# BAMresearch/McSAS

Hardware: AMD Instinct MI355X
Metric: MC accept/reject steps/sec (whole node) (higher is better)
Workload: dtype f64; 1 GPU; Sphere, synthetic 512 q-points x 400 contribs, 50 reps on this rank (50 in all), 20000 MC steps per chain per launch, convergenceCriterion=0, one analysis on the chip at a time; reps_total=50, reps_per_gpu=50, ranks_seen=1, streams=1, exec_mode=pipeline, waves_per_chain=1, q_per_lane=8, window=192, launches=108, cached_rows=True

## Files before the change

### mcsas_amd/csrc/pipe_gram.h

```cpp
#pragma once
#include "pipe_layout.h"

namespace mcsas {

#define PIPE_LDS_BARRIER() do { asm volatile("s_waitcnt lgkmcnt(0)" ::: "memory"); __builtin_amdgcn_s_barrier(); asm volatile("" ::: "memory"); } while (0)

typedef double v4f64 __attribute__((ext_vector_type(4)));
typedef double v2f64 __attribute__((ext_vector_type(2)));


template <int T>
__device__ __forceinline__ void pipe_gram_store(int tsel, int idx, double sum, int W, MCSAS_GLOBAL double *gout, MCSAS_GLOBAL double *scal_sub = nullptr) {
    int ti = 0, tgi = 0, tgj = 0;
#pragma unroll
    for (int gi = 0; gi < T; ++gi)
#pragma unroll
        for (int gj = gi; gj < T; ++gj) { if (ti == tsel) { tgi = gi; tgj = gj; } ++ti; }
    const int i = 4 * (idx >> 6) + ((idx & 63) >> 4), j = idx & 15;
    const int ar = 16 * tgi + i, kc = 16 * tgj + j;
    if (ar < W && kc < W) {
        gout[(size_t)ar * W + kc] = sum;
        if (scal_sub && ar == kc) scal_sub[ar * 4 + 2] = sum;
    }
}

template <int QPL, int T, bool PACK>
__device__ __forceinline__ void pipe_gram_mfma_lds(const double *drows, int dstr, int nvalid, const double *lw, int gw,
                                                   v4f64 (&acc)[PACK ? 2 : T * (T + 1) / 2]) {
    const int lane = threadIdx.x & 63;
    const int m = lane & 15, kk = lane >> 4;
    constexpr int NT = PACK ? 2 : T * (T + 1) / 2;
    constexpr int NL = PACK ? 3 : T;
    constexpr int SLICE = 64 * QPL / PIPE_WAVES;
    static_assert(SLICE >= 8, "too many waves for this q count");
    const int qs = gw * SLICE + kk * 2;
#pragma unroll
    for (int i = 0; i < NT; ++i) acc[i] = (v4f64){0., 0., 0., 0.};
    const double *rowp[NL];
    bool rowok[NL];
#pragma unroll
    for (int gi = 0; gi < NL; ++gi) {
        const int rr = PACK ? (gi == 0 ? m : gi == 1 ? 8 + m : (m < 8 ? m : m + 8)) : 16 * gi + m;
        rowok[gi] = rr < nvalid;
        rowp[gi] = drows + (size_t)(rowok[gi] ? rr : 0) * dstr + qs;
    }
#pragma unroll
    for (int sp = 0; sp < SLICE / 8; ++sp) {
        v2f64 av[NL], bv[NL];
        const v2f64 wv = *reinterpret_cast<const v2f64 *>(lw + qs + 8 * sp);
#pragma unroll
        for (int gi = 0; gi < NL; ++gi) {
            const v2f64 x = *reinterpret_cast<const v2f64 *>(rowp[gi] + 8 * sp);
            av[gi] = rowok[gi] ? x : (v2f64){0., 0.};
            bv[gi] = av[gi] * wv;
        }
        if constexpr (PACK) {
            acc[0] = __builtin_amdgcn_mfma_f64_16x16x4f64(av[0].x, bv[1].x, acc[0], 0, 0, 0);
            acc[1] = __builtin_amdgcn_mfma_f64_16x16x4f64(av[2].x, bv[2].x, acc[1], 0, 0, 0);
            acc[0] = __builtin_amdgcn_mfma_f64_16x16x4f64(av[0].y, bv[1].y, acc[0], 0, 0, 0);
            acc[1] = __builtin_amdgcn_mfma_f64_16x16x4f64(av[2].y, bv[2].y, acc[1], 0, 0, 0);
        } else {
            int ti = 0;
#pragma unroll
            for (int gi = 0; gi < T; ++gi)
#pragma unroll
                for (int gj = gi; gj < T; ++gj) {
                    acc[ti] = __builtin_amdgcn_mfma_f64_16x16x4f64(av[gi].x, bv[gj].x, acc[ti], 0, 0, 0);
                    acc[ti] = __builtin_amdgcn_mfma_f64_16x16x4f64(av[gi].y, bv[gj].y, acc[ti], 0, 0, 0);
                    ++ti;
                }
        }
    }
}

__device__ __forceinline__ void pipe_gram_store_pack(int tsel, int idx, double sum, MCSAS_GLOBAL double *gout, MCSAS_GLOBAL double *scal_sub) {
    const int i = 4 * (idx >> 6) + ((idx & 63) >> 4), j = idx & 15;
    if (tsel == 0) {
        gout[(size_t)i * 24 + 8 + j] = sum;
        if (i == 8 + j) scal_sub[i * 4 + 2] = sum;
    } else if ((i < 8) == (j < 8)) {
        const int ar = i < 8 ? i : i + 8, kc = j < 8 ? j : j + 8;
        gout[(size_t)ar * 24 + kc] = sum;
        if (ar == kc) scal_sub[ar * 4 + 2] = sum;
    }
}

template <int QPL, int T, bool PACK>
__device__ __forceinline__ void pipe_prod_gram_lds_t(const double *drows, int dstr, int W, int nvalid, const double *lw,
                                                     double *gred, MCSAS_GLOBAL double *gout, MCSAS_GLOBAL double *scal_sub) {
    const int tid = threadIdx.x, lane = tid & 63, wave = __builtin_amdgcn_readfirstlane(tid >> 6);
    constexpr int NT = PACK ? 2 : T * (T + 1) / 2;
    v4f64 acc[NT];
    pipe_gram_mfma_lds<QPL, T, PACK>(drows, dstr, nvalid, lw, wave, acc);
    constexpr int TPR = PIPE_GRAM_TILES_PER_ROUND;
#pragma unroll
    for (int r0 = 0; r0 < NT; r0 += TPR) {
#pragma unroll
        for (int u = 0; u < TPR; ++u)
            if (r0 + u < NT) {
#pragma unroll
                for (int r = 0; r < 4; ++r) gred[((size_t)(wave * TPR + u) * 4 + r) * 64 + lane] = acc[r0 + u < NT ? r0 + u : 0][r];
            }
        PIPE_LDS_BARRIER();
        {
            const int u = tid >> 8, idx = tid & 255;
            const int tsel = r0 + u;
            if (tsel < NT) {
                double sum = 0.;
#pragma unroll
                for (int v = 0; v < PIPE_WAVES; ++v) sum += gred[(size_t)(v * TPR + u) * 256 + idx];
                if constexpr (PACK) pipe_gram_store_pack(tsel, idx, sum, gout, scal_sub);
                else pipe_gram_store<T>(tsel, idx, sum, W, gout, scal_sub);
            }
        }
        if (r0 + TPR < NT) PIPE_LDS_BARRIER();
    }
}

template <int QPL>
__device__ __forceinline__ void pipe_prod_gram_lds(const double *drows, int dstr, int W, int nvalid, const double *lw,
                                                   double *gred, MCSAS_GLOBAL double *gout, MCSAS_GLOBAL double *scal_sub) {
    if (W == 24) { pipe_prod_gram_lds_t<QPL, 2, true>(drows, dstr, W, nvalid, lw, gred, gout, scal_sub); return; }
    switch ((W + 15) >> 4) {
        case 1: pipe_prod_gram_lds_t<QPL, 1, false>(drows, dstr, W, nvalid, lw, gred, gout, scal_sub); break;
        case 2: pipe_prod_gram_lds_t<QPL, 2, false>(drows, dstr, W, nvalid, lw, gred, gout, scal_sub); break;
        case 3: pipe_prod_gram_lds_t<QPL, 3, false>(drows, dstr, W, nvalid, lw, gred, gout, scal_sub); break;
        default: pipe_prod_gram_lds_t<QPL, 4, false>(drows, dstr, W, nvalid, lw, gred, gout, scal_sub); break;
    }
}

#ifdef MCSAS_TUNING

template <int QPL, int T, bool PACK>
__device__ __forceinline__ void pipe_gram_units(const MCSAS_GLOBAL double *drows, int qpad, int nvalid, const double *lw, int gw,
                                                int u0, int u1, v4f64 (&acc)[PIPE_GRAM_NT_MAX]) {
    static_assert(T <= 2, "at most two 16-row groups per sub-window");
    const int lane = threadIdx.x & 63;
    const int m = lane & 15, kk = lane >> 4;
    constexpr int NL = PACK ? 3 : T;
    constexpr int SLICE = 64 * QPL / PIPE_WAVES;
    static_assert(SLICE >= 8, "too many waves for this q count");
    const int qs = gw * SLICE + kk * 2;
    if (u0 == 0) {
#pragma unroll
        for (int i = 0; i < PIPE_GRAM_NT_MAX; ++i) acc[i] = (v4f64){0., 0., 0., 0.};
    }
    const MCSAS_GLOBAL double *rowp[NL];
    bool rowok[NL];
#pragma unroll
    for (int gi = 0; gi < NL; ++gi) {
        const int rr = PACK ? (gi == 0 ? m : gi == 1 ? 8 + m : (m < 8 ? m : m + 8)) : 16 * gi + m;
        rowok[gi] = rr < nvalid;
        rowp[gi] = drows + (size_t)(rowok[gi] ? rr : 0) * qpad + qs;
    }
    v2f64 cur[NL], nxt[NL];
#pragma unroll
    for (int gi = 0; gi < NL; ++gi) cur[gi] = *(const MCSAS_GLOBAL v2f64 *)(rowp[gi] + 8 * u0);
    for (int u = u0; u < u1; ++u) {
        const int un = u + 1 < u1 ? u + 1 : u;
#pragma unroll
        for (int gi = 0; gi < NL; ++gi) nxt[gi] = *(const MCSAS_GLOBAL v2f64 *)(rowp[gi] + 8 * un);
        const v2f64 wv = *reinterpret_cast<const v2f64 *>(lw + qs + 8 * u);
        v2f64 av[NL], bv[NL];
#pragma unroll
        for (int gi = 0; gi < NL; ++gi) {
            av[gi] = rowok[gi] ? cur[gi] : (v2f64){0., 0.};
            bv[gi] = av[gi] * wv;
        }
        if constexpr (PACK) {
            acc[0] = __builtin_amdgcn_mfma_f64_16x16x4f64(av[0].x, bv[1].x, acc[0], 0, 0, 0);
            acc[1] = __builtin_amdgcn_mfma_f64_16x16x4f64(av[2].x, bv[2].x, acc[1], 0, 0, 0);
            acc[0] = __builtin_amdgcn_mfma_f64_16x16x4f64(av[0].y, bv[1].y, acc[0], 0, 0, 0);
            acc[1] = __builtin_amdgcn_mfma_f64_16x16x4f64(av[2].y, bv[2].y, acc[1], 0, 0, 0);
        } else {
            int ti = 0;
#pragma unroll
            for (int gi = 0; gi < T; ++gi)
#pragma unroll
                for (int gj = gi; gj < T; ++gj) { acc[ti] = __builtin_amdgcn_mfma_f64_16x16x4f64(av[gi].x, bv[gj].x, acc[ti], 0, 0, 0); ++ti; }
            ti = 0;
#pragma unroll
            for (int gi = 0; gi < T; ++gi)
#pragma unroll
                for (int gj = gi; gj < T; ++gj) { acc[ti] = __builtin_amdgcn_mfma_f64_16x16x4f64(av[gi].y, bv[gj].y, acc[ti], 0, 0, 0); ++ti; }
        }
#pragma unroll
        for (int gi = 0; gi < NL; ++gi) cur[gi] = nxt[gi];
    }
}

constexpr int PIPE_GRAM_PREF = 12;
template <int T, bool PACK> struct PipeGramScheme {
    static constexpr int NL = PACK ? 3 : T;
    static constexpr int UCAP = PIPE_GRAM_PREF / NL;
};
template <int QPL, int T, bool PACK>
__device__ __forceinline__ void pipe_gram_fetch(const MCSAS_GLOBAL double *drows, int qpad, int nvalid, int gw, int u0, int n,
                                                v2f64 (&G)[PIPE_GRAM_PREF]) {
    const int lane = threadIdx.x & 63;
    const int m = lane & 15, kk = lane >> 4;
    constexpr int NL = PipeGramScheme<T, PACK>::NL, UCAP = PipeGramScheme<T, PACK>::UCAP;
    constexpr int SLICE = 64 * QPL / PIPE_WAVES;
    const int qs = gw * SLICE + kk * 2;
#pragma unroll
    for (int gi = 0; gi < NL; ++gi) {
        const int rr = PACK ? (gi == 0 ? m : gi == 1 ? 8 + m : (m < 8 ? m : m + 8)) : 16 * gi + m;
        const MCSAS_GLOBAL double *rowp = drows + (size_t)(rr < nvalid ? rr : 0) * qpad + qs;
#pragma unroll
        for (int i = 0; i < UCAP; ++i) {
            const int u = u0 + (i < n ? i : n - 1);
            G[i * NL + gi] = *(const MCSAS_GLOBAL v2f64 *)(rowp + 8 * u);
        }
    }
}
template <int QPL, int T, bool PACK>
__device__ __forceinline__ void pipe_gram_consume(const v2f64 (&G)[PIPE_GRAM_PREF], int nvalid, const double *lw, int gw, int u0, int n,
                                                  v4f64 (&acc)[PIPE_GRAM_NT_MAX]) {
    const int lane = threadIdx.x & 63;
    const int m = lane & 15, kk = lane >> 4;
    constexpr int NL = PipeGramScheme<T, PACK>::NL, UCAP = PipeGramScheme<T, PACK>::UCAP;
    constexpr int SLICE = 64 * QPL / PIPE_WAVES;
    const int qs = gw * SLICE + kk * 2;
    if (u0 == 0) {
#pragma unroll
        for (int i = 0; i < PIPE_GRAM_NT_MAX; ++i) acc[i] = (v4f64){0., 0., 0., 0.};
    }
    bool rowok[NL];
#pragma unroll
    for (int gi = 0; gi < NL; ++gi) {
        const int rr = PACK ? (gi == 0 ? m : gi == 1 ? 8 + m : (m < 8 ? m : m + 8)) : 16 * gi + m;
        rowok[gi] = rr < nvalid;
    }
#pragma unroll
    for (int i = 0; i < UCAP; ++i)
        if (i < n) {
            const v2f64 wv = *reinterpret_cast<const v2f64 *>(lw + qs + 8 * (u0 + i));
            v2f64 av[NL], bv[NL];
#pragma unroll
            for (int gi = 0; gi < NL; ++gi) {
                av[gi] = rowok[gi] ? G[i * NL + gi] : (v2f64){0., 0.};
                bv[gi] = av[gi] * wv;
            }
            if constexpr (PACK) {
                acc[0] = __builtin_amdgcn_mfma_f64_16x16x4f64(av[0].x, bv[1].x, acc[0], 0, 0, 0);
                acc[1] = __builtin_amdgcn_mfma_f64_16x16x4f64(av[2].x, bv[2].x, acc[1], 0, 0, 0);
                acc[0] = __builtin_amdgcn_mfma_f64_16x16x4f64(av[0].y, bv[1].y, acc[0], 0, 0, 0);
                acc[1] = __builtin_amdgcn_mfma_f64_16x16x4f64(av[2].y, bv[2].y, acc[1], 0, 0, 0);
            } else {
                int ti = 0;
#pragma unroll
                for (int gi = 0; gi < T; ++gi)
#pragma unroll
                    for (int gj = gi; gj < T; ++gj) { acc[ti] = __builtin_amdgcn_mfma_f64_16x16x4f64(av[gi].x, bv[gj].x, acc[ti], 0, 0, 0); ++ti; }
                ti = 0;
#pragma unroll
                for (int gi = 0; gi < T; ++gi)
#pragma unroll
                    for (int gj = gi; gj < T; ++gj) { acc[ti] = __builtin_amdgcn_mfma_f64_16x16x4f64(av[gi].y, bv[gj].y, acc[ti], 0, 0, 0); ++ti; }
            }
        }
}

__device__ __forceinline__ int pipe_gram_tiles(int W) { return W == 24 ? 2 : (W <= 16 ? 1 : 3); }

__device__ __forceinline__ void pipe_gram_park(const v4f64 (&acc)[PIPE_GRAM_NT_MAX], int nt, double *gred, int wave, int lane) {
#pragma unroll
    for (int ti = 0; ti < PIPE_GRAM_NT_MAX; ++ti)
        if (ti < nt) {
#pragma unroll
            for (int r = 0; r < 4; ++r) gred[((size_t)(wave * PIPE_GRAM_NT_MAX + ti) * 4 + r) * 64 + lane] = acc[ti][r];
        }
}

__device__ __forceinline__ void pipe_gram_sum_store(int W, const double *gred, MCSAS_GLOBAL double *gout, MCSAS_GLOBAL double *scal_sub) {
    const int tid = threadIdx.x;
    const int nt = pipe_gram_tiles(W);
    for (int e = tid; e < nt * 256; e += PIPE_BLOCK) {
        const int ti = e >> 8, idx = e & 255;
        double sum = 0.;
#pragma unroll
        for (int v = 0; v < PIPE_WAVES; ++v) sum += gred[(size_t)(v * PIPE_GRAM_NT_MAX + ti) * 256 + idx];
        const int i = 4 * (idx >> 6) + ((idx & 63) >> 4), j = idx & 15;
        int ar = -1, kc = -1;
        if (W == 24) {
            if (ti == 0) { ar = i; kc = 8 + j; }
            else if ((i < 8) == (j < 8)) { ar = i < 8 ? i : i + 8; kc = j < 8 ? j : j + 8; }
        } else {
            const int tgi = ti == 2 ? 1 : 0, tgj = ti == 0 ? 0 : 1;
            ar = 16 * tgi + i; kc = 16 * tgj + j;
        }
        if (ar >= 0 && ar < W && kc < W) {
            gout[(size_t)ar * W + kc] = sum;
            if (ar == kc) scal_sub[ar * 4 + 2] = sum;
        }
    }
}
#endif

}
```

### mcsas_amd/csrc/pipe_prod.h

```cpp
#pragma once
#include "pipe_rowq.h"
#include <type_traits>

namespace mcsas {

#define PIPE_PIN_ROW(arr) do { _Pragma("unroll") for (int j_ = 0; j_ < QPL; ++j_) asm volatile("" : "+v"(arr[j_])); } while (0)

#ifdef MCSAS_STAMPS
#define PIPE_TL_SLOT(pa, i) (pa).timeline[((size_t)blockIdx.x * 8 + (threadIdx.x >> 6)) * PIPE_TL_WORDS + 4 + (i)]
#define PIPE_TL_PUT(pa, t, i, val) do { if ((pa).timeline && (t) - 1 == (pa).timeline_tick && (threadIdx.x & 63) == 0) PIPE_TL_SLOT(pa, i) = (val); } while (0)
#define PIPE_TL_CLOCK(var) const uint64_t var = wall_clock64()
#else
#define PIPE_TL_PUT(pa, t, i, val) do {} while (0)
#define PIPE_TL_CLOCK(var) do {} while (0)
#endif
#define PIPE_TL_WRITE(pa, t, i) PIPE_TL_PUT(pa, t, i, wall_clock64())
#define PIPE_TLX_MARK(pa, t, i) PIPE_TL_WRITE(pa, t, 18 + (i))
#define PIPE_TL_MARK(pa, t, i) PIPE_TL_WRITE(pa, t, i)

template <int M> constexpr bool pipe_light_model_v = Contrib<M>::ROW_CLASS == 0;
template <int M>
__device__ __forceinline__ double pipe_point_intensity(const Contrib<M> &c, double q, double q3inv, const double *tab) {
    if constexpr (M == MCSAS_MODEL_SPHERE) return c.fast ? c.intensity_fast(q, q3inv) : c.intensity(q, tab);
    else return c.intensity(q, tab);
}

template <int QPL>
__device__ __forceinline__ void load_row_pairs(const MCSAS_GLOBAL double *row, int lane, double (&r)[QPL]) {
    if constexpr (QPL >= 2) {
#pragma unroll
        for (int c = 0; c < QPL / 2; ++c) {
            const v2f64 v = *(const MCSAS_GLOBAL v2f64 *)(row + 128 * c + 2 * lane);
            r[2 * c] = v.x; r[2 * c + 1] = v.y;
        }
    } else {
        r[0] = row[lane];
    }
}
template <int QPL>
__device__ __forceinline__ void load_row_pairs_lds(const double *row, int lane, double (&r)[QPL]) {
    if constexpr (QPL >= 2) {
#pragma unroll
        for (int c = 0; c < QPL / 2; ++c) {
            const v2f64 v = *reinterpret_cast<const v2f64 *>(row + 128 * c + 2 * lane);
            r[2 * c] = v.x; r[2 * c + 1] = v.y;
        }
    } else {
        r[0] = row[lane];
    }
}

template <int M, int QPL, bool RQ>
__device__ __forceinline__ void pipe_prod_block(const PipeArgs &pa, const PipeHot &hot, double *lds, int rep, int by, int gy, int t) {
    const ChainArgs &a = pa.c;
    const int tid = threadIdx.x, lane = tid & 63, wave = tid >> 6;
    constexpr int WPB = PIPE_BLOCK / 64;
    const int N = hot.n_contrib, P = hot.n_active, qpad = hot.qpad, Kb = hot.kb;
    const int64_t max_iter = hot.max_iter;
    constexpr int QTB = (QPL * 64 + PIPE_BLOCK - 1) / PIPE_BLOCK;
    double tq[QTB], tw[QTB], twI[QTB], tq3[QTB];
#pragma unroll
    for (int x = 0; x < QTB; ++x) {
        const int i = tid + PIPE_BLOCK * x < qpad ? tid + PIPE_BLOCK * x : 0;
        tq[x] = glb(hot.q)[i]; tw[x] = glb(hot.w)[i]; twI[x] = glb(hot.wI)[i]; tq3[x] = glb(hot.q3inv)[i];
    }
    PIPE_TL_CLOCK(c_entry);
    const PipeSnap sn = load_snap(&hot.chains[rep].snap[t & 1]);
    const bool own = sn.alive && t >= sn.t_init;
    if (!own && !(RQ && pa.g.help)) return;
    PIPE_TL_CLOCK(c_snap);

    double *lq = lds, *lw = lds + qpad, *lwI = lds + 2 * qpad, *lq3 = lds + 3 * qpad, *tab = lds + 4 * qpad;
#pragma unroll
    for (int x = 0; x < QTB; ++x) {
        const int i = tid + PIPE_BLOCK * x;
        if (i < qpad) { lq[i] = tq[x]; lw[i] = tw[x]; lwI[i] = twI[x]; lq3[i] = tq3[x]; }
    }
    PIPE_TL_CLOCK(c_tab);
    Contrib<M>::fill_table(a.model, tab, tid, PIPE_BLOCK);
    if (tid == 0) {
        *reinterpret_cast<int32_t *>(lds + pa.g.gram_off + 16) = 0;
        *reinterpret_cast<int32_t *>(lds + pa.g.gram_off) = 0;
    }
    __syncthreads();
    PIPE_TL_CLOCK(c_bar);
    PIPE_TL_PUT(pa, t, 22, c_entry); PIPE_TL_PUT(pa, t, 23, c_snap); PIPE_TL_PUT(pa, t, 24, c_tab); PIPE_TL_PUT(pa, t, 25, c_bar);
    const QTables qt = make_qtables<M>(a.model, lq, lq3, tab);
    if constexpr (RQ) { pipe_prod_rowq<M, QPL>(pa, hot, lds, qt, rep, by, gy, t, sn, own); return; }
    auto rset = glb(a.rset) + (size_t)rep * N * P;
    auto cache = glb(a.cache) + (size_t)rep * a.cache_rows * qpad;
    const DrawSource src{a.replay ? a.replay + (size_t)rep * a.replay_len : nullptr, a.replay_len, a.seed,
                         (uint32_t)(a.rep_offset + rep)};
    auto slot_of = glb(pa.slot_of) + (size_t)rep * N;
    auto stage = glb(pa.stage_slot) + (size_t)rep * 2 * Kb;
    auto row_valid = glb(pa.row_valid) + (size_t)rep * N;
    const int gw = by * WPB + wave, nw = gy * WPB;

    if (t == sn.t_init) {
        for (int i = tid + by * PIPE_BLOCK; i < N; i += PIPE_BLOCK * gy) { slot_of[i] = i; row_valid[i] = 1; }
        for (int i = tid + by * PIPE_BLOCK; i < 2 * Kb; i += PIPE_BLOCK * gy) stage[i] = N + i;
        int ovf = 0;
        for (int nb = 0; nb < N; nb += nw * WAVE) {
            const int n = nb + lane * nw + gw;
            double row[MCSAS_MAX_ACTIVE] = {0., 0., 0., 0.};
            if (n < N) {
#pragma unroll
                for (int p = 0; p < MCSAS_MAX_ACTIVE; ++p)
                    if (p < P) {
                        if (a.start_from_min) row[p] = a.start_value[p];
                        else {
                            double u = src.at(sn.init_base + (uint64_t)p * N + n, ovf);
                            row[p] = gen_transform(a.gen_kind[p], u) * (a.gen_hi[p] - a.gen_lo[p]) + a.gen_lo[p];
                        }
                        rset[(size_t)n * P + p] = row[p];
                    }
            } else {
#pragma unroll
                for (int p = 0; p < MCSAS_MAX_ACTIVE; ++p) row[p] = a.gen_lo[p] > 0. ? a.gen_lo[p] : 1e-9;
            }
            Contrib<M> mine;
            mine.prepare(a.model, row);
            for (int l = 0; l < WAVE; ++l) {
                const int nn = nb + l * nw + gw;
                if (nn >= N) break;
                const Contrib<M> c = mine.bcast(__builtin_amdgcn_readfirstlane(l));
                double it[QPL];
                RowEval<M, QPL>::run(c, qt, lane, it);
#pragma unroll
                for (int j = 0; j < QPL; ++j) cache[(size_t)nn * qpad + lane + WAVE * j] = it[j];
            }
        }
        if (__any(ovf) && lane == 0) atomicOr(&pa.chains[rep].overflow, 1);
        return;
    }

    if (MCSAS_TUNE_BITS(a) & 16) return;
    if constexpr (pipe_light_model_v<M>) if (pa.g.overlap || pa.g.gram_lds) {
        const int W = pa.g.w, nsb = pa.g.sub_per_block, BR = nsb * W;
        const int buf = t & 1;
        const int64_t w = (int64_t)t - sn.t_init - 1;
        const int64_t sb0 = w * Kb + (int64_t)by * BR;
        auto dwin = glb(pa.dwin) + ((size_t)rep * 2 + buf) * Kb * qpad;
        auto scal = glb(pa.scal) + ((size_t)rep * 2 + buf) * Kb * 4;
        auto pval = glb(pa.pval) + ((size_t)rep * 2 + buf) * Kb * MCSAS_MAX_ACTIVE;
        auto povf = glb(pa.povf) + ((size_t)rep * 2 + buf) * Kb;
        auto gwin = glb(pa.gwin) + ((size_t)rep * 2 + buf) * Kb * W;
        double *gred = lds + pa.g.gram_off + 16;
        const bool no_gram = MCSAS_TUNE_BITS(a) & 64;
        const bool lazy = pa.g.lazy_rows;
        PIPE_TLX_MARK(pa, t, 0);
        constexpr int CON = PIPE_PROP_DOUBLES;
        static_assert(sizeof(Contrib<M>) <= 8 * (CON - 1) && sizeof(Contrib<M>) % 8 == 0, "Contrib record");
        int32_t *stl = reinterpret_cast<int32_t *>(gred);
        double *scon = gred + 64;
        auto stale_push = [&](int r, const Contrib<M> &c) {
            const int e = atomicAdd(&stl[0], 1);
            stl[1 + e] = r;
            double tmp[CON] = {};
            __builtin_memcpy(tmp, &c, sizeof(Contrib<M>));
#pragma unroll
            for (int i = 0; i < (int)(sizeof(Contrib<M>) / 8); ++i) scon[e * CON + i] = tmp[i];
        };
        auto stale_refresh = [&]() {
            PIPE_LDS_BARRIER();
            const int nst = stl[0];
            for (int i = 0; i < nst; ++i) {
                const int r = stl[1 + i];
                Contrib<M> c;
                {
                    double tmp[CON];
#pragma unroll
                    for (int x = 0; x < (int)(sizeof(Contrib<M>) / 8); ++x) tmp[x] = scon[i * CON + x];
                    __builtin_memcpy(&c, tmp, sizeof(Contrib<M>));
                }
#pragma unroll
                for (int x = 0; x < QTB; ++x) {
                    const int iq = tid + PIPE_BLOCK * x;
                    if (iq < qpad) cache[(size_t)r * qpad + iq] = pipe_point_intensity<M>(c, lq[iq], lq3[iq], tab);
                }
                if (tid == 0) row_valid[r] = 1;
            }
            if (nst) __syncthreads();
            else PIPE_LDS_BARRIER();
        };
        auto nvalid_of = [&](int ss) {
            const int64_t left = max_iter - (w * Kb + (int64_t)(by * nsb + ss) * W);
            return left >= W ? W : (left > 0 ? (int)left : 0);
        };
        if (pa.g.gram_lds) {
            const int dstr = qpad + PIPE_DROW_PAD;
            double *dbuf = lds + pa.g.drow_off;
            double *prec = lds + pa.g.rec_off;
            int32_t *claim = reinterpret_cast<int32_t *>(lds + pa.g.gram_off);
            auto take = [&]() {
                int v = 0;
                if (lane == 0) v = __hip_atomic_fetch_add(claim, 1, __ATOMIC_RELAXED, __HIP_MEMORY_SCOPE_WORKGROUP);
                return __builtin_amdgcn_readfirstlane(v);
            };
            int kc = take();
            const int kk = tid & 63;
            const int64_t sl = sb0 + kk;
            const bool prop_thr = tid < BR, old_thr = lazy && tid >= 64 && tid - 64 < BR && sl < max_iter;
            const int rk = (int)(sl % N);
            double prow[MCSAS_MAX_ACTIVE] = {0., 0., 0., 0.};
            int stale_r = -1, pov = 0;
            if (old_thr) {
                const int v = row_valid[rk];
#pragma unroll
                for (int p = 0; p < MCSAS_MAX_ACTIVE; ++p) if (p < P) prow[p] = rset[(size_t)rk * P + p];
                if (!v) stale_r = rk;
            }
#pragma unroll
            for (int p = 0; p < MCSAS_MAX_ACTIVE; ++p)
                if (p < P) {
                    double u = 0.5;
                    if (prop_thr && sl < max_iter) u = src.at(sn.step_base + (uint64_t)sl * P + p, pov);
                    const double pv = gen_transform(a.gen_kind[p], u) * (a.gen_hi[p] - a.gen_lo[p]) + a.gen_lo[p];
                    if (!old_thr) prow[p] = pv;
                }
            Contrib<M> prop;
            prop.prepare(a.model, prow);
            PIPE_TLX_MARK(pa, t, 1);
            if (prop_thr) {
                double tmp[CON] = {};
                __builtin_memcpy(tmp, &prop, sizeof(Contrib<M>));
#pragma unroll
                for (int i = 0; i < (int)(sizeof(Contrib<M>) / 8); ++i) prec[kk * CON + i] = tmp[i];
                if (!lazy) {
                    int32_t *slots = reinterpret_cast<int32_t *>(prec + kk * CON + CON - 1);
                    slots[0] = slot_of[rk]; slots[1] = stage[buf * Kb + by * BR + kk];
                }
                const int k = by * BR + kk;
#pragma unroll
                for (int p = 0; p < MCSAS_MAX_ACTIVE; ++p) if (p < P) pval[k * MCSAS_MAX_ACTIVE + p] = prow[p];
                povf[k] = pov;
            }
            if (stale_r >= 0) stale_push(stale_r, prop);
            if (lazy) stale_refresh();
            else PIPE_LDS_BARRIER();
            PIPE_TLX_MARK(pa, t, 2);
            PIPE_TLX_MARK(pa, t, 3);
            const int r0 = (int)(sb0 % N);
            auto oslot_of = [&](int k) {
                if (lazy) return r0 + k < N ? r0 + k : r0 + k - N;
                return __builtin_amdgcn_readfirstlane(reinterpret_cast<const int32_t *>(prec + k * CON + CON - 1)[0]);
            };
            double ocur[QPL], onext[QPL];
            {
                const auto orow0 = cache + (size_t)oslot_of(kc < BR ? kc : BR - 1) * qpad + lane;
#pragma unroll
                for (int j = 0; j < QPL; ++j) ocur[j] = orow0[WAVE * j];
            }
            PIPE_PIN_ROW(ocur);
#ifdef MCSAS_STAMPS
            int nmine = 0;
#endif
            for (int ss = 0; ss < nsb; ++ss) {
                while (kc < (ss + 1) * W) {
                    const int kn = take();
                    const int k = by * BR + kc;
                    Contrib<M> cnew;
                    int sslot = 0;
                    {
                        Contrib<M> cl;
                        double tmp[CON];
#pragma unroll
                        for (int i = 0; i < (int)(sizeof(Contrib<M>) / 8); ++i) tmp[i] = prec[kc * CON + i];
                        __builtin_memcpy(&cl, tmp, sizeof(Contrib<M>));
                        cnew = cl.bcast(0);
                        if (!lazy) sslot = __builtin_amdgcn_readfirstlane(reinterpret_cast<const int32_t *>(prec + kc * CON + CON - 1)[1]);
                    }
                    double d[QPL], nwv[QPL];
                    {
                        const auto orow = cache + (size_t)oslot_of(kn < BR ? kn : kc) * qpad + lane;
#pragma unroll
                        for (int j = 0; j < QPL; ++j) onext[j] = orow[WAVE * j];
                    }
                    const auto nrow = cache + (size_t)sslot * qpad + lane;
                    const auto dr = dwin + (size_t)k * qpad + lane;
                    double *dl = dbuf + (size_t)(kc - ss * W) * dstr + lane;
                    RowEval<M, QPL>::run(cnew, qt, lane, nwv);
#ifdef MCSAS_STAMPS
                    if (nmine < 4) { PIPE_PIN_ROW(nwv); PIPE_TL_MARK(pa, t, 4 + 2 * nmine); }
#endif
                    PIPE_PIN_ROW(ocur); PIPE_PIN_ROW(onext); PIPE_PIN_ROW(nwv);
                    double s1 = 0., s2 = 0.;
#pragma unroll
                    for (int j = 0; j < QPL; ++j) {
                        const int iq = lane + WAVE * j;
                        if (!lazy) nrow[WAVE * j] = nwv[j];
                        d[j] = nwv[j] - ocur[j];
                        dr[WAVE * j] = d[j];
                        dl[WAVE * j] = d[j];
                        s1 = fma(lw[iq], d[j], s1); s2 = fma(lwI[iq], d[j], s2);
                    }
                    const double ae = wave_sum2_split(s1, s2, lane);
                    if (lane < 2) scal[(size_t)k * 4 + lane] = ae;
#pragma unroll
                    for (int j = 0; j < QPL; ++j) ocur[j] = onext[j];
#ifdef MCSAS_STAMPS
                    if (nmine < 4) PIPE_TL_MARK(pa, t, 5 + 2 * nmine);
                    ++nmine;
#endif
                    kc = kn;
                }
                PIPE_TL_MARK(pa, t, 2 * (ss < 4 ? ss : 3));
                if (!no_gram) PIPE_LDS_BARRIER();
                const int nvalid = nvalid_of(ss);
                if (nvalid > 0 && !no_gram)
                    pipe_prod_gram_lds<QPL>(dbuf, dstr, W, nvalid, lw, gred, gwin + (size_t)(by * nsb + ss) * W * W,
                                            scal + (size_t)(by * BR + ss * W) * 4);
                PIPE_TL_MARK(pa, t, 2 * (ss < 4 ? ss : 3) + 1);
            }
            PIPE_TL_MARK(pa, t, 17);
            return;
        }
#ifdef MCSAS_TUNING
#include "pipe_prod_overlap.inc"
#endif
        PIPE_TL_MARK(pa, t, 17);
        return;
    }

}

}
```

Baseline: 309.4 million MC steps/s.

## Split waves into gram and row roles to overlap next-row evaluation with gram MFMA

During the per-sub-window gram reduction, half the waves now run the MFMA work over two q-slices each while the other half evaluate the next contribution row and hold its delta in registers. The held row is written into the LDS buffer only after the last reduction barrier. The MFMA loop also gains software prefetch of the next slice's operands, with a scheduling barrier between load and compute. The intent is to hide row-evaluation latency behind gram compute and cut load stalls, at the cost of more register pressure and more complex barrier and role logic.

Result: faster. 313.6 million MC steps/s, median of 6 (+1.3%).

```diff
diff --git a/mcsas_amd/csrc/pipe_gram.h b/mcsas_amd/csrc/pipe_gram.h
--- a/mcsas_amd/csrc/pipe_gram.h
+++ b/mcsas_amd/csrc/pipe_gram.h
@@ -24,18 +24,21 @@
     }
 }
 
-template <int QPL, int T, bool PACK>
-__device__ __forceinline__ void pipe_gram_mfma_lds(const double *drows, int dstr, int nvalid, const double *lw, int gw,
-                                                   v4f64 (&acc)[PACK ? 2 : T * (T + 1) / 2]) {
+template <int QPL, int T, bool PACK, int R0, int RN, int NS>
+__device__ __forceinline__ void pipe_gram_mfma_lds(const double *drows, int dstr, int nvalid, const double *lw, int gw, v4f64 (&acc)[NS][RN]) {
     const int lane = threadIdx.x & 63;
     const int m = lane & 15, kk = lane >> 4;
     constexpr int NT = PACK ? 2 : T * (T + 1) / 2;
     constexpr int NL = PACK ? 3 : T;
-    constexpr int SLICE = 64 * QPL / PIPE_WAVES;
+    constexpr int SLICE = 64 * QPL / PIPE_WAVES, STEPS = SLICE / 8;
+    constexpr int SSTR = (PIPE_WAVES / 2) * SLICE;
     static_assert(SLICE >= 8, "too many waves for this q count");
+    static_assert(R0 >= 0 && RN >= 1 && R0 + RN <= NT && (!PACK || (R0 == 0 && RN == 2)) && (NS == 1 || NS == 2), "tiles and slices of the sub-window");
     const int qs = gw * SLICE + kk * 2;
 #pragma unroll
-    for (int i = 0; i < NT; ++i) acc[i] = (v4f64){0., 0., 0., 0.};
+    for (int s = 0; s < NS; ++s)
+#pragma unroll
+        for (int i = 0; i < RN; ++i) acc[s][i] = (v4f64){0., 0., 0., 0.};
     const double *rowp[NL];
     bool rowok[NL];
 #pragma unroll
@@ -44,31 +47,60 @@
         rowok[gi] = rr < nvalid;
         rowp[gi] = drows + (size_t)(rowok[gi] ? rr : 0) * dstr + qs;
     }
-#pragma unroll
-    for (int sp = 0; sp < SLICE / 8; ++sp) {
-        v2f64 av[NL], bv[NL];
-        const v2f64 wv = *reinterpret_cast<const v2f64 *>(lw + qs + 8 * sp);
-#pragma unroll
-        for (int gi = 0; gi < NL; ++gi) {
-            const v2f64 x = *reinterpret_cast<const v2f64 *>(rowp[gi] + 8 * sp);
-            av[gi] = rowok[gi] ? x : (v2f64){0., 0.};
-            bv[gi] = av[gi] * wv;
-        }
+    auto fetch = [&](int sp, v2f64 (&x)[NS][NL], v2f64 (&wv)[NS]) {
+#pragma unroll
+        for (int s = 0; s < NS; ++s) {
+            wv[s] = *reinterpret_cast<const v2f64 *>(lw + qs + s * SSTR + 8 * sp);
+#pragma unroll
+            for (int gi = 0; gi < NL; ++gi) x[s][gi] = *reinterpret_cast<const v2f64 *>(rowp[gi] + s * SSTR + 8 * sp);
+        }
+    };
+    v2f64 cur[NS][NL], cw[NS];
+    fetch(0, cur, cw);
+#pragma unroll
+    for (int sp = 0; sp < STEPS; ++sp) {
+        v2f64 nxt[NS][NL], nw[NS];
+        if (sp + 1 < STEPS) fetch(sp + 1, nxt, nw);
+        __builtin_amdgcn_sched_barrier(0);
+        v2f64 av[NS][NL], bv[NS][NL];
+#pragma unroll
+        for (int s = 0; s < NS; ++s)
+#pragma unroll
+            for (int gi = 0; gi < NL; ++gi) {
+                av[s][gi] = rowok[gi] ? cur[s][gi] : (v2f64){0., 0.};
+                bv[s][gi] = av[s][gi] * cw[s];
+            }
         if constexpr (PACK) {
-            acc[0] = __builtin_amdgcn_mfma_f64_16x16x4f64(av[0].x, bv[1].x, acc[0], 0, 0, 0);
-            acc[1] = __builtin_amdgcn_mfma_f64_16x16x4f64(av[2].x, bv[2].x, acc[1], 0, 0, 0);
-            acc[0] = __builtin_amdgcn_mfma_f64_16x16x4f64(av[0].y, bv[1].y, acc[0], 0, 0, 0);
-            acc[1] = __builtin_amdgcn_mfma_f64_16x16x4f64(av[2].y, bv[2].y, acc[1], 0, 0, 0);
+#pragma unroll
+            for (int s = 0; s < NS; ++s) acc[s][0] = __builtin_amdgcn_mfma_f64_16x16x4f64(av[s][0].x, bv[s][1].x, acc[s][0], 0, 0, 0);
+#pragma unroll
+            for (int s = 0; s < NS; ++s) acc[s][1] = __builtin_amdgcn_mfma_f64_16x16x4f64(av[s][2].x, bv[s][2].x, acc[s][1], 0, 0, 0);
+#pragma unroll
+            for (int s = 0; s < NS; ++s) acc[s][0] = __builtin_amdgcn_mfma_f64_16x16x4f64(av[s][0].y, bv[s][1].y, acc[s][0], 0, 0, 0);
+#pragma unroll
+            for (int s = 0; s < NS; ++s) acc[s][1] = __builtin_amdgcn_mfma_f64_16x16x4f64(av[s][2].y, bv[s][2].y, acc[s][1], 0, 0, 0);
         } else {
             int ti = 0;
 #pragma unroll
             for (int gi = 0; gi < T; ++gi)
 #pragma unroll
                 for (int gj = gi; gj < T; ++gj) {
-                    acc[ti] = __builtin_amdgcn_mfma_f64_16x16x4f64(av[gi].x, bv[gj].x, acc[ti], 0, 0, 0);
-                    acc[ti] = __builtin_amdgcn_mfma_f64_16x16x4f64(av[gi].y, bv[gj].y, acc[ti], 0, 0, 0);
+                    if (ti >= R0 && ti < R0 + RN) {
+#pragma unroll
+                        for (int s = 0; s < NS; ++s) acc[s][ti - R0] = __builtin_amdgcn_mfma_f64_16x16x4f64(av[s][gi].x, bv[s][gj].x, acc[s][ti - R0], 0, 0, 0);
+#pragma unroll
+                        for (int s = 0; s < NS; ++s) acc[s][ti - R0] = __builtin_amdgcn_mfma_f64_16x16x4f64(av[s][gi].y, bv[s][gj].y, acc[s][ti - R0], 0, 0, 0);
+                    }
                     ++ti;
                 }
+        }
+        if (sp + 1 < STEPS) {
+#pragma unroll
+            for (int s = 0; s < NS; ++s) {
+                cw[s] = nw[s];
+#pragma unroll
+                for (int gi = 0; gi < NL; ++gi) cur[s][gi] = nxt[s][gi];
+            }
         }
     }
 }
@@ -85,47 +117,68 @@
     }
 }
 
-template <int QPL, int T, bool PACK>
-__device__ __forceinline__ void pipe_prod_gram_lds_t(const double *drows, int dstr, int W, int nvalid, const double *lw,
-                                                     double *gred, MCSAS_GLOBAL double *gout, MCSAS_GLOBAL double *scal_sub) {
+template <int QPL, int T, bool PACK, int R0, class Behind>
+__device__ __forceinline__ void pipe_gram_round(const double *drows, int dstr, int W, int nvalid, const double *lw, double *gred,
+                                                MCSAS_GLOBAL double *gout, MCSAS_GLOBAL double *scal_sub, bool split, bool matrix, Behind &&behind) {
     const int tid = threadIdx.x, lane = tid & 63, wave = __builtin_amdgcn_readfirstlane(tid >> 6);
     constexpr int NT = PACK ? 2 : T * (T + 1) / 2;
-    v4f64 acc[NT];
-    pipe_gram_mfma_lds<QPL, T, PACK>(drows, dstr, nvalid, lw, wave, acc);
-    constexpr int TPR = PIPE_GRAM_TILES_PER_ROUND;
-#pragma unroll
-    for (int r0 = 0; r0 < NT; r0 += TPR) {
-#pragma unroll
-        for (int u = 0; u < TPR; ++u)
-            if (r0 + u < NT) {
-#pragma unroll
-                for (int r = 0; r < 4; ++r) gred[((size_t)(wave * TPR + u) * 4 + r) * 64 + lane] = acc[r0 + u < NT ? r0 + u : 0][r];
-            }
+    constexpr int TPR = PIPE_GRAM_TILES_PER_ROUND, RN = NT - R0 < TPR ? NT - R0 : TPR;
+    constexpr int MW = PIPE_WAVES / 2;
+    if (matrix) {
+        auto park = [&](int slot, const v4f64 (&acc)[RN]) {
+#pragma unroll
+            for (int u = 0; u < RN; ++u)
+#pragma unroll
+                for (int r = 0; r < 4; ++r) gred[((size_t)(slot * TPR + u) * 4 + r) * 64 + lane] = acc[u][r];
+        };
+        if (split) {
+            v4f64 acc[2][RN];
+            pipe_gram_mfma_lds<QPL, T, PACK, R0, RN, 2>(drows, dstr, nvalid, lw, wave, acc);
+            park(wave, acc[0]); park(wave + MW, acc[1]);
+        } else {
+            v4f64 acc[1][RN];
+            pipe_gram_mfma_lds<QPL, T, PACK, R0, RN, 1>(drows, dstr, nvalid, lw, wave, acc);
+            park(wave, acc[0]);
+        }
+    }
+    PIPE_LDS_BARRIER();
+    if (R0 + TPR >= NT && !matrix) behind();
+    {
+        const int u = tid >> 8, idx = tid & 255;
+        const int tsel = R0 + u;
+        if (tsel < NT) {
+            double sum = 0.;
+#pragma unroll
+            for (int v = 0; v < PIPE_WAVES; ++v) sum += gred[(size_t)(v * TPR + u) * 256 + idx];
+            if constexpr (PACK) pipe_gram_store_pack(tsel, idx, sum, gout, scal_sub);
+            else pipe_gram_store<T>(tsel, idx, sum, W, gout, scal_sub);
+        }
+    }
+    if constexpr (R0 + TPR < NT) {
         PIPE_LDS_BARRIER();
-        {
-            const int u = tid >> 8, idx = tid & 255;
-            const int tsel = r0 + u;
-            if (tsel < NT) {
-                double sum = 0.;
-#pragma unroll
-                for (int v = 0; v < PIPE_WAVES; ++v) sum += gred[(size_t)(v * TPR + u) * 256 + idx];
-                if constexpr (PACK) pipe_gram_store_pack(tsel, idx, sum, gout, scal_sub);
-                else pipe_gram_store<T>(tsel, idx, sum, W, gout, scal_sub);
-            }
-        }
-        if (r0 + TPR < NT) PIPE_LDS_BARRIER();
-    }
-}
-
-template <int QPL>
+        pipe_gram_round<QPL, T, PACK, R0 + TPR>(drows, dstr, W, nvalid, lw, gred, gout, scal_sub, split, matrix, behind);
+    }
+}
+
+template <int QPL, int T, bool PACK, class Behind>
+__device__ __forceinline__ void pipe_prod_gram_lds_t(const double *drows, int dstr, int W, int nvalid, const double *lw,
+                                                     double *gred, MCSAS_GLOBAL double *gout, MCSAS_GLOBAL double *scal_sub,
+                                                     bool split, Behind &&behind) {
+    const int wave = __builtin_amdgcn_readfirstlane(threadIdx.x >> 6);
+    const bool matrix = !split || wave < PIPE_WAVES / 2;
+    pipe_gram_round<QPL, T, PACK, 0>(drows, dstr, W, nvalid, lw, gred, gout, scal_sub, split, matrix, behind);
+}
+
+template <int QPL, class Behind>
 __device__ __forceinline__ void pipe_prod_gram_lds(const double *drows, int dstr, int W, int nvalid, const double *lw,
-                                                   double *gred, MCSAS_GLOBAL double *gout, MCSAS_GLOBAL double *scal_sub) {
-    if (W == 24) { pipe_prod_gram_lds_t<QPL, 2, true>(drows, dstr, W, nvalid, lw, gred, gout, scal_sub); return; }
+                                                   double *gred, MCSAS_GLOBAL double *gout, MCSAS_GLOBAL double *scal_sub,
+                                                   bool split, Behind &&behind) {
+    if (W == 24) { pipe_prod_gram_lds_t<QPL, 2, true>(drows, dstr, W, nvalid, lw, gred, gout, scal_sub, split, behind); return; }
     switch ((W + 15) >> 4) {
-        case 1: pipe_prod_gram_lds_t<QPL, 1, false>(drows, dstr, W, nvalid, lw, gred, gout, scal_sub); break;
-        case 2: pipe_prod_gram_lds_t<QPL, 2, false>(drows, dstr, W, nvalid, lw, gred, gout, scal_sub); break;
-        case 3: pipe_prod_gram_lds_t<QPL, 3, false>(drows, dstr, W, nvalid, lw, gred, gout, scal_sub); break;
-        default: pipe_prod_gram_lds_t<QPL, 4, false>(drows, dstr, W, nvalid, lw, gred, gout, scal_sub); break;
+#define PIPE_GRAM_CASE(T) case T: if constexpr ((2 * T - 1) * QPL <= PIPE_MAX_ROW_DOUBLES) pipe_prod_gram_lds_t<QPL, T, false>(drows, dstr, W, nvalid, lw, gred, gout, scal_sub, split, behind); break;
+        PIPE_GRAM_CASE(1) PIPE_GRAM_CASE(2) PIPE_GRAM_CASE(3) PIPE_GRAM_CASE(4)
+#undef PIPE_GRAM_CASE
+        default: break;
     }
 }
 
diff --git a/mcsas_amd/csrc/pipe_prod.h b/mcsas_amd/csrc/pipe_prod.h
--- a/mcsas_amd/csrc/pipe_prod.h
+++ b/mcsas_amd/csrc/pipe_prod.h
@@ -255,61 +255,77 @@
 #ifdef MCSAS_STAMPS
             int nmine = 0;
 #endif
+            const bool roles = !(MCSAS_TUNE_BITS(a) & (1 << 17));
+            const bool row_wave = roles && __builtin_amdgcn_readfirstlane(wave) >= WPB / 2;
+            auto eval_row = [&](int sr, auto hold, double (&d)[QPL]) {
+                const int kn = take();
+                const int k = by * BR + kc;
+                Contrib<M> cnew;
+                int sslot = 0;
+                {
+                    Contrib<M> cl;
+                    double tmp[CON];
+#pragma unroll
+                    for (int i = 0; i < (int)(sizeof(Contrib<M>) / 8); ++i) tmp[i] = prec[kc * CON + i];
+                    __builtin_memcpy(&cl, tmp, sizeof(Contrib<M>));
+                    cnew = cl.bcast(0);
+                    if (!lazy) sslot = __builtin_amdgcn_readfirstlane(reinterpret_cast<const int32_t *>(prec + kc * CON + CON - 1)[1]);
+                }
+                double nwv[QPL];
+                {
+                    const auto orow = cache + (size_t)oslot_of(kn < BR ? kn : kc) * qpad + lane;
+#pragma unroll
+                    for (int j = 0; j < QPL; ++j) onext[j] = orow[WAVE * j];
+                }
+                const auto nrow = cache + (size_t)sslot * qpad + lane;
+                const auto dr = dwin + (size_t)k * qpad + lane;
+                double *dl = dbuf + (size_t)(kc - sr * W) * dstr + lane;
+                RowEval<M, QPL>::run(cnew, qt, lane, nwv);
+#ifdef MCSAS_STAMPS
+                if (nmine < 4) { PIPE_PIN_ROW(nwv); PIPE_TL_MARK(pa, t, 4 + 2 * nmine); }
+#endif
+                PIPE_PIN_ROW(ocur); PIPE_PIN_ROW(onext); PIPE_PIN_ROW(nwv);
+                double s1 = 0., s2 = 0.;
+#pragma unroll
+                for (int j = 0; j < QPL; ++j) {
+                    const int iq = lane + WAVE * j;
+                    if (!lazy) nrow[WAVE * j] = nwv[j];
+                    d[j] = nwv[j] - ocur[j];
+                    dr[WAVE * j] = d[j];
+                    if constexpr (!decltype(hold)::value) dl[WAVE * j] = d[j];
+                    s1 = fma(lw[iq], d[j], s1); s2 = fma(lwI[iq], d[j], s2);
+                }
+                const double ae = wave_sum2_split(s1, s2, lane);
+                if (lane < 2) scal[(size_t)k * 4 + lane] = ae;
+#pragma unroll
+                for (int j = 0; j < QPL; ++j) ocur[j] = onext[j];
+#ifdef MCSAS_STAMPS
+                if (nmine < 4) PIPE_TL_MARK(pa, t, 5 + 2 * nmine);
+                ++nmine;
+#endif
+                kc = kn;
+            };
             for (int ss = 0; ss < nsb; ++ss) {
                 while (kc < (ss + 1) * W) {
-                    const int kn = take();
-                    const int k = by * BR + kc;
-                    Contrib<M> cnew;
-                    int sslot = 0;
-                    {
-                        Contrib<M> cl;
-                        double tmp[CON];
-#pragma unroll
-                        for (int i = 0; i < (int)(sizeof(Contrib<M>) / 8); ++i) tmp[i] = prec[kc * CON + i];
-                        __builtin_memcpy(&cl, tmp, sizeof(Contrib<M>));
-                        cnew = cl.bcast(0);
-                        if (!lazy) sslot = __builtin_amdgcn_readfirstlane(reinterpret_cast<const int32_t *>(prec + kc * CON + CON - 1)[1]);
-                    }
-                    double d[QPL], nwv[QPL];
-                    {
-                        const auto orow = cache + (size_t)oslot_of(kn < BR ? kn : kc) * qpad + lane;
-#pragma unroll
-                        for (int j = 0; j < QPL; ++j) onext[j] = orow[WAVE * j];
-                    }
-                    const auto nrow = cache + (size_t)sslot * qpad + lane;
-                    const auto dr = dwin + (size_t)k * qpad + lane;
-                    double *dl = dbuf + (size_t)(kc - ss * W) * dstr + lane;
-                    RowEval<M, QPL>::run(cnew, qt, lane, nwv);
-#ifdef MCSAS_STAMPS
-                    if (nmine < 4) { PIPE_PIN_ROW(nwv); PIPE_TL_MARK(pa, t, 4 + 2 * nmine); }
-#endif
-                    PIPE_PIN_ROW(ocur); PIPE_PIN_ROW(onext); PIPE_PIN_ROW(nwv);
-                    double s1 = 0., s2 = 0.;
-#pragma unroll
-                    for (int j = 0; j < QPL; ++j) {
-                        const int iq = lane + WAVE * j;
-                        if (!lazy) nrow[WAVE * j] = nwv[j];
-                        d[j] = nwv[j] - ocur[j];
-                        dr[WAVE * j] = d[j];
-                        dl[WAVE * j] = d[j];
-                        s1 = fma(lw[iq], d[j], s1); s2 = fma(lwI[iq], d[j], s2);
-                    }
-                    const double ae = wave_sum2_split(s1, s2, lane);
-                    if (lane < 2) scal[(size_t)k * 4 + lane] = ae;
-#pragma unroll
-                    for (int j = 0; j < QPL; ++j) ocur[j] = onext[j];
-#ifdef MCSAS_STAMPS
-                    if (nmine < 4) PIPE_TL_MARK(pa, t, 5 + 2 * nmine);
-                    ++nmine;
-#endif
-                    kc = kn;
+                    double d[QPL];
+                    eval_row(ss, std::false_type{}, d);
                 }
                 PIPE_TL_MARK(pa, t, 2 * (ss < 4 ? ss : 3));
                 if (!no_gram) PIPE_LDS_BARRIER();
                 const int nvalid = nvalid_of(ss);
-                if (nvalid > 0 && !no_gram)
+                if (nvalid > 0 && !no_gram) {
+                    double dheld[QPL];
+                    int kheld = -1;
+                    if (row_wave && kc < BR && kc < (ss + 2) * W) { kheld = kc; eval_row(ss + 1, std::true_type{}, dheld); }
                     pipe_prod_gram_lds<QPL>(dbuf, dstr, W, nvalid, lw, gred, gwin + (size_t)(by * nsb + ss) * W * W,
-                                            scal + (size_t)(by * BR + ss * W) * 4);
+                                            scal + (size_t)(by * BR + ss * W) * 4, roles, [&]() {
+                                                if (kheld >= 0) {
+                                                    double *dl = dbuf + (size_t)(kheld - (ss + 1) * W) * dstr + lane;
+#pragma unroll
+                                                    for (int j = 0; j < QPL; ++j) dl[WAVE * j] = dheld[j];
+                                                }
+                                            });
+                }
                 PIPE_TL_MARK(pa, t, 2 * (ss < 4 ? ss : 3) + 1);
             }
             PIPE_TL_MARK(pa, t, 17);
```
